# nnethercott/hannoy

Hardware: AMD Instinct MI355X
Metric: vectors indexed/sec (build) + recall@10, 1M x 768 Cosine M=16 efC=100 (higher is better)
Workload: dtype f32

## Files before the change

### hannoy_amd/csrc/hny_host.cpp

```cpp
#include "../../include/hannoy_amd.h"
#include "hny_internal.h"
#include "hny_rust_sort.h"

#include <malloc.h>
#include <algorithm>
#include <array>
#include <atomic>
#include <mutex>
#include <chrono>
#include <cmath>
#include <cstdarg>
#include <cstdio>
#include <cstdlib>
#include <cstring>
#include <functional>
#include <iterator>
#include <memory>
#include <numeric>
#include <string>
#include <thread>
#include <type_traits>
#include <utility>
#include <vector>

// ... 295 lines not shown
  bool gaps_done = false;
  bool from_update = false;
  uint64_t n_done0 = 0;
  uint32_t up_layers = 1;
  std::vector<uint32_t> entry_points;
  std::vector<uint64_t> rec_first;
  std::vector<uint32_t> rec_item_t;
  std::vector<uint8_t> rec_layer_t;
  std::vector<int32_t> upper_idx;
  uint32_t max_level = 0, n_upper = 0;
  LaunchShape shape{64, 1};
  double frac = 0.0;
  uint32_t bmax = 0;
  int device = 0;
  hipStream_t stream = nullptr;
  std::vector<hipEvent_t> sync_evs;
  size_t sync_used = 0;
  size_t pos = 0;
  uint64_t n_done = 0, n_batches = 0;
  hny_batch cur{};
  bool in_batch = false, finalized = false;
  GraphDev g{};
  DevBuf<unsigned char> d_rows, d_level;
  DevBuf<float> d_norms, d_l0_dist, d_up_dist;
  DevBuf<int> d_upper_idx;
  DevBuf<u32> d_l0_ids, d_l0_cnt, d_up_ids, d_up_cnt, d_order, d_eps, d_bits, d_vlog, d_cand_n,
      d_seg_start, d_nseg, d_deferred, d_deferred_b, d_fin_cnt0, d_fin_cntu, d_d0_ids, d_du_ids;
  DevBuf<unsigned char> d_has_vec, d_deleted;
  DevBuf<u64> d_old_recs, d_lkey_a, d_lkey_b, d_perm_a, d_perm_b;
  DevBuf<u32> d_gap_bitmap, d_gap_bm;
  DevBuf<u64> d_gap_keys, d_gap_sorted;
  int gap_grid = 0;
  DevBuf<u32> d_eps0;
  DevBuf<u32> d_pool_retry, d_pool_retry2, d_pool_ctr;
  DevBuf<u64> d_heap_c, d_heap_r;
  uint32_t heap_grid = 0, heap_c_cap = 0, heap_r_cap = 0, pool_ctr_used = 0;
  uint32_t heap_grid1 = 0, heap_c_cap1 = 0;
  u64 *heap_c_ptr = nullptr;
  struct ExportBufs : ExportSlots {
    std::thread th;
    void join() {
      if (th.joinable()) th.join();
    }
    void drop() {
      join();
      drop_all();
    }
    ~ExportBufs() { drop(); }
  } xbuf;
  bool will_export = true;
  std::vector<uint32_t> item_slot;
  uint64_t n_items = 0;
  std::unique_ptr<IngestPipe> qpipe;
  uint64_t nrec_bound = 0, nbr_bound = 0;
  bool locality = true;
  u32 *h_l0 = nullptr, *h_up = nullptr, *h_cnt0 = nullptr, *h_cntu = nullptr;
  DevBuf<u64> d_stats, d_stats_scratch, d_sel, d_cand, d_res_global;
  DevBuf<u64> d_ops;
  struct { u64 *p = nullptr; size_t n = 0; } d_keys_a, d_keys_b, d_vals_a, d_vals_b;
  DevBuf<unsigned char> d_sort_tmp;
  size_t sort_tmp_bytes = 0;
  uint32_t walk_slots = 0, bits_words = 0, log_cap = 0, rcap = 0, max_batch = 0;
  Knobs knobs{};
  uint32_t xcd_tile = 0, prune_xcd_tile = 0, walk_resident = 0;
  uint64_t top_layer_nodes = 0;
  StageRows stage{0, 0};
// ... 116 lines not shown
  for (uint32_t v : set)
    if (c <= v) {
      s.lpr = (int)l;
      s.nch = (int)v;
      return HNY_OK;
    }
  return fail(HNY_ERR_UNSUPPORTED, "dim %u needs more than 16 chunks per lane (max f32 dim 4096)", dim);
}

int mclass_of(int metric) {
  switch (metric) {
    case HNY_COSINE: return MC_DOT;
    case HNY_EUCLIDEAN: return MC_L2;
    case HNY_MANHATTAN: return MC_L1;
    default: return MC_BIN;
  }
}

uint32_t cap_of(const hny_builder *b, uint32_t layer_or_level) {
  return layer_or_level == 0 ? b->o.M0 : b->o.M;
}

int env_int(const char *name, int dflt) {
  const char *v = getenv(name);
  return v && *v ? atoi(v) : dflt;
}

Knobs knobs_from_env() {
  Knobs k{};
  k.no_fast = env_int("HNY_NO_FAST", 0) != 0;
  k.no_rb = env_int("HNY_NO_RB", 0) != 0;
  k.rb_one = env_int("HNY_RB_ONE", 1) != 0;
  k.prune_n8 = env_int("HNY_PRUNE_N8", 1) != 0;
  k.walk_slots = env_int("HNY_WALK_SLOTS", HNY_KNOB_UNSET);
  k.xcd_tile = env_int("HNY_XCD_TILE", HNY_KNOB_UNSET);
  k.prune_xcd_tile = env_int("HNY_PRUNE_XCD_TILE", HNY_KNOB_UNSET);
  k.walk_resident = env_int("HNY_WALK_RESIDENT", HNY_KNOB_UNSET);
  k.visited_log = env_int("HNY_VISITED_LOG", HNY_KNOB_UNSET);
  k.vis_slots = env_int("HNY_VIS_SLOTS", HNY_KNOB_UNSET);
  k.stage_bytes = env_int("HNY_STAGE_BYTES", HNY_KNOB_UNSET);
  k.no_locality = env_int("HNY_NO_LOCALITY", 0) != 0;
  k.heap_small_cap = env_int("HNY_HEAP_SMALL_CAP", HNY_KNOB_UNSET);
  k.vis_buckets = env_int("HNY_VIS_BUCKETS", HNY_KNOB_UNSET);
  return k;
}

int upload_rows(const void *vectors, size_t stride, size_t vbytes, uint64_t n, uint32_t row_stride,
                unsigned char *dst, hipStream_t st, const uint32_t *slots = nullptr, uint64_t n_slots = 0) {
  if (!slots) n_slots = n;
  if (!slots && stride == row_stride && vbytes == row_stride) {
    HIP_TRY(hipMemcpyAsync(dst, vectors, (size_t)n * row_stride, hipMemcpyHostToDevice, st));
    HIP_TRY(hipStreamSynchronize(st));
    return HNY_OK;
  }
  const size_t chunk_rows = std::max<size_t>(1, (64u << 20) / row_stride);
  std::vector<unsigned char> stage(chunk_rows * row_stride);
  uint64_t r = 0;
  for (uint64_t s0 = 0; s0 < n_slots; s0 += chunk_rows) {
    size_t cnt = (size_t)std::min<uint64_t>(chunk_rows, n_slots - s0);
    std::fill(stage.begin(), stage.begin() + cnt * row_stride, 0);
    for (; r < n && (slots ? slots[r] : r) < s0 + cnt; r++)
      memcpy(&stage[((slots ? slots[r] : r) - s0) * row_stride], (const unsigned char *)vectors + r * stride, vbytes);
    HIP_TRY(hipMemcpyAsync(dst + s0 * row_stride, stage.data(), cnt * row_stride,
                           hipMemcpyHostToDevice, st));
    HIP_TRY(hipStreamSynchronize(st));
  }
// ... 116 lines not shown
    if (j.out_codes)
      HIP_TRY(hipMemcpyAsync((unsigned char *)j.out_codes + r0 * vb, p.d_codes[k], (size_t)cnt * vb, hipMemcpyDeviceToHost, st));
    if (j.out_hdrs)
      HIP_TRY(hipMemcpyAsync((unsigned char *)j.out_hdrs + r0 * hb, p.d_hdrs[k], (size_t)cnt * hb, hipMemcpyDeviceToHost, st));
  }
  return HNY_OK;
}

int check_f32_rows(uint32_t dim, uint64_t n, const void *vectors, size_t stride) {
  if (dim == 0) return fail(HNY_ERR_INVALID_DIM, "dim must be > 0");
  if (n && !vectors) return fail(HNY_ERR_INVALID_ARG, "null f32 vectors");
  if (n && stride < (size_t)dim * 4)
    return fail(HNY_ERR_INVALID_DIM, "stride %zu < %zu bytes of f32 for dim %u", stride, (size_t)dim * 4, dim);
  if (n && stride % 4) return fail(HNY_ERR_INVALID_ARG, "f32 stride %zu is not a multiple of 4", stride);
  return HNY_OK;
}

int reset_graph(hny_builder *b) {
  hipStream_t st = b->stream;
  HIP_TRY(hnyk_fill_u32(b->d_l0_ids.p, HNY_SENT, b->d_l0_ids.n, st));
  HIP_TRY(hipMemsetAsync(b->d_l0_cnt.p, 0, b->d_l0_cnt.n * 4, st));
  HIP_TRY(hipMemsetAsync(b->d_l0_dist.p, 0, b->d_l0_dist.n * 4, st));
  if (b->d_up_ids.n) {
    HIP_TRY(hnyk_fill_u32(b->d_up_ids.p, HNY_SENT, b->d_up_ids.n, st));
    HIP_TRY(hipMemsetAsync(b->d_up_cnt.p, 0, b->d_up_cnt.n * 4, st));
    HIP_TRY(hipMemsetAsync(b->d_up_dist.p, 0, b->d_up_dist.n * 4, st));
  }
  HIP_TRY(hipMemsetAsync(b->d_stats.p, 0, ST_COUNT * 8, st));
  HIP_TRY(hipMemsetAsync(b->d_bits.p, 0, b->d_bits.n * 4, st));
  b->pos = 0;
  b->n_done = b->n_done0;
  b->n_batches = 0;
  b->in_batch = false;
  b->finalized = false;
  b->gaps_done = false;
  b->ev_used = 0;
  b->n_walk_dispatch = 0;
  b->sync_used = 0;
  b->t_build0 = now_s();
  return HNY_OK;
}

int use_device(int device) {
  int ndev = 0;
  if (hipGetDeviceCount(&ndev) != hipSuccess || ndev == 0)
    return fail(HNY_ERR_NO_DEVICE, "no HIP device (this library has no CPU path)");
  if (device >= 0) HIP_TRY(hipSetDevice(device));
  return HNY_OK;
}

size_t group_end(const hny_builder *b, size_t pos) {
  size_t e = pos;
  while (e < b->order.size() && b->order_level[e] == b->order_level[pos]) e++;
  return e;
}

inline uint32_t rec_mask_of(const hny_builder *b, uint32_t s) {
  if (b->deleted[s]) return 0u;
  uint32_t m = b->old_mask[s];
  if (b->ins_level[s] >= 0) m |= (2u << b->ins_level[s]) - 1u;
  return m;
}
template <class F>
inline void for_each_record(const hny_builder *b, uint32_t s, F &&fn) {
  for (uint32_t m = rec_mask_of(b, s), l = 0; m; m >>= 1, l++)
    if (m & 1) fn(l, l == 0 ? (size_t)s : (size_t)b->upper_idx[s] * b->up_layers + (l - 1));
// ... 618 lines not shown
}
static uint32_t walk_slots_default(const WalkForm &plain) { return 256u * 4u * (uint32_t)plain.waves_per_simd; }
static int plan_launch(hny_builder *b, const Knobs &knobs) {
  const hny_build_opts &o = b->o;
  const uint32_t n = b->n, n16 = b->g.n16;
  const Knobs &k = b->knobs = knobs;
  b->g.metric = o.metric;
  b->g.M = o.M;
  b->g.M0 = o.M0;
  b->g.incremental = b->incremental ? 1 : 0;
  b->g.x86_order = o.x86_order ? 1 : 0;
  b->rcap = res_capacity(o.ef_construction, (uint32_t)b->entry_points.size(), n, b->top_layer_nodes, HNY_RES_GLOBAL_MAX);
  b->rb_one = rb_one_of(o.ef_construction, b->entry_points.size(), b->top_layer_nodes, o.M);
  b->walk_slots = walk_slots_default(plain_walk_form(b, b->rcap, k.no_rb != 0));
  b->walk_slots = (uint32_t)std::min<int64_t>(std::max(1, knob_or(k.walk_slots, (int)b->walk_slots)), 65536);
  b->xcd_tile = (u32)std::max(0, knob_or(k.xcd_tile, n16 * 16u >= 1024u ? 512 : 0));
  b->prune_xcd_tile = (u32)std::max(0, knob_or(k.prune_xcd_tile, 512));
  const bool long_row_rb = n16 * 16u >= 1024u && plain_walk_form(b, b->rcap, false).rc != 0;
  const int resident = knob_or(k.walk_resident, long_row_rb ? 12 : 0);
  if (resident < 0 || resident > 256)
    return fail(HNY_ERR_INVALID_ARG, "HNY_WALK_RESIDENT=%d: 0 (= HNY_WALK_SLOTS) .. 256 waves per CU", resident);
  b->walk_resident = 256u * (u32)resident;
  b->bits_words = (n + 31) / 32 + 1;
  b->log_cap = (uint32_t)std::max(1024, knob_or(k.visited_log, 16384));
  b->locality = !k.no_locality;
  int rpg = 64 / b->shape.lpr;
  int sl = (int)((u32)std::max(0, knob_or(k.stage_bytes, 24576)) / (n16 * 16u));
  if (sl > HNY_MAX_CAP) sl = HNY_MAX_CAP;
  b->stage.wg = sl / rpg * rpg;
  b->stage.n8 = (int)std::min<uint32_t>(HNY_MAX_CAP, std::max<uint32_t>(1, 6144u / (n16 * 16u)));
  b->apply_form = hnyk_apply_form(b->g, b->shape, k);
  return HNY_OK;
}
static int plan_sizes(hny_builder *b, const CreatePlan &P) {
  const hny_build_opts &o = b->o;
  b->max_batch = 1;
  b->max_ops = 2;
  b->sel_words = 2;
  for (size_t pos = 0; pos < b->order.size();) {
    size_t e = group_end(b, pos);
    uint32_t L = b->order_level[pos];
    uint64_t bs = std::min<uint64_t>(b->bmax, e - pos);
    uint64_t cs = cap_of(b, L);
    b->max_batch = std::max<uint32_t>(b->max_batch, (uint32_t)bs);
    b->max_ops = std::max<size_t>(b->max_ops, (size_t)(bs * (L + 1) * cs * 2));
    b->sel_words = std::max<size_t>(b->sel_words, (size_t)(bs * (L + 1) * (cs + 1)));
    pos = e;
  }
  if (b->max_ops >= (1ull << HNY_SEQ_BITS))
    return fail(HNY_ERR_UNSUPPORTED,
                "batch_max %u too large for M0 %u: %zu link ops per batch >= 2^%d (pass batch_max <= %u; the schedule "
                "is part of the result, so it is never shrunk silently)",
                b->bmax, o.M0, b->max_ops, HNY_SEQ_BITS, (uint32_t)((1ull << (HNY_SEQ_BITS - 1)) / std::max(o.M0, 2 * o.M) / 2));
  if (int rc = plan_launch(b, knobs_from_env())) return rc;
  if (o.M0 > HNY_MAX_CAP && b->shape.nch > 8 && P.inc && !P.inc->load_only)
    return fail(HNY_ERR_UNSUPPORTED, "M0 %u > %d: an incremental build needs the workgroup kernels (rows <= 8 KB)",
                o.M0, HNY_MAX_CAP);
  return HNY_OK;
}

static int alloc_device(hny_builder *b, const CreatePlan &P) {
  const hny_build_opts &o = b->o;
  hipStream_t st = b->stream;
  const uint32_t n = b->n;
  const size_t nn = std::max<uint32_t>(n, 1);
  const size_t no = std::max<size_t>(b->order.size(), 1);
  const size_t nup = (size_t)b->n_upper * b->up_layers;
  const uint32_t row_stride = b->g.n16 * 16;
  HIP_TRY(b->d_rows.alloc(nn * row_stride));
  HIP_TRY(b->d_level.alloc(nn));
  HIP_TRY(b->d_upper_idx.alloc(nn));
  if (has_norms(o.metric)) HIP_TRY(b->d_norms.alloc(nn));
  HIP_TRY(b->d_l0_ids.alloc(nn * o.M0));
  HIP_TRY(b->d_l0_dist.alloc(nn * o.M0));
  HIP_TRY(b->d_l0_cnt.alloc(nn));
  HIP_TRY(b->d_up_ids.alloc(nup * o.M));
  HIP_TRY(b->d_up_dist.alloc(nup * o.M));
  HIP_TRY(b->d_up_cnt.alloc(nup));
  HIP_TRY(b->d_order.alloc(no));
  HIP_TRY(b->d_fin_cnt0.alloc(nn));
  HIP_TRY(b->d_fin_cntu.alloc(std::max<size_t>(nup, 1)));
  HIP_TRY(hipHostMalloc((void **)&b->h_l0, nn * o.M0 * 4));
  HIP_TRY(hipHostMalloc((void **)&b->h_cnt0, nn * 4));
  HIP_TRY(hipHostMalloc((void **)&b->h_up, std::max<size_t>(nup * o.M, 1) * 4));
  HIP_TRY(hipHostMalloc((void **)&b->h_cntu, std::max<size_t>(nup, 1) * 4));
  HIP_TRY(b->d_eps.alloc(std::max<size_t>(64, b->entry_points.size())));
  HIP_TRY(b->d_stats.alloc(ST_COUNT));
  const uint32_t slots = std::min<uint32_t>(b->walk_slots, std::max<uint32_t>(b->max_batch, 256));
  b->walk_slots = slots;
  HIP_TRY(b->d_bits.alloc((size_t)slots * b->bits_words));
  HIP_TRY(b->d_vlog.alloc((size_t)slots * b->log_cap));
  HIP_TRY(b->d_sel.alloc(b->sel_words));
  const size_t cand_rows = std::max<uint32_t>(b->max_batch, 256);
  if (b->rcap > HNY_RES_LDS_MAX) {
    if (b->apply_form.kind == APPLY_WAVE)
      return fail(HNY_ERR_UNSUPPORTED, "a result set of %u entries needs the workgroup prune kernels (no x86_order, rows <= 8 KB)", b->rcap);
    if ((cand_rows + slots) * (size_t)b->rcap * 8 > ((size_t)24 << 30))
      return fail(HNY_ERR_UNSUPPORTED, "result sets of %u entries for %zu batch members exceed the 24 GB set aside for them; "
                  "pass a smaller batch_max", b->rcap, cand_rows);
    HIP_TRY(b->d_res_global.alloc((size_t)slots * b->rcap));
  }
  HIP_TRY(b->d_cand.alloc(cand_rows * b->rcap));
  HIP_TRY(b->d_cand_n.alloc(cand_rows));
  HIP_TRY(b->d_ops.alloc(4 * b->max_ops));
  b->d_keys_a.p = b->d_ops.p;
  b->d_keys_b.p = b->d_ops.p + b->max_ops;
  b->d_vals_a.p = b->d_ops.p + 2 * b->max_ops;
  b->d_vals_b.p = b->d_ops.p + 3 * b->max_ops;
  b->d_keys_a.n = b->d_keys_b.n = b->d_vals_a.n = b->d_vals_b.n = b->max_ops;
  HIP_TRY(b->d_seg_start.alloc(b->max_ops));
  HIP_TRY(b->d_nseg.alloc(4 + 16 + 8 * 16));
  HIP_TRY(b->d_lkey_a.alloc(cand_rows));
  HIP_TRY(b->d_lkey_b.alloc(cand_rows));
  HIP_TRY(b->d_perm_a.alloc(cand_rows));
  HIP_TRY(b->d_perm_b.alloc(cand_rows));
  HIP_TRY(b->d_eps0.alloc(cand_rows));
  {
    const uint64_t c_full = (uint64_t)n + 1 + eps_cap_of(b);
    b->heap_r_cap = b->rcap + 1;
    if (b->d_ops.n >= c_full) {
      b->heap_c_cap = (uint32_t)std::min<uint64_t>(c_full, 0xFFFFFFFFull);
      b->heap_grid = (uint32_t)std::min<uint64_t>(std::min<uint64_t>(slots, 512), b->d_ops.n / c_full);
      b->heap_c_ptr = b->d_ops.p;
    } else {
      b->heap_c_cap = (uint32_t)std::min<uint64_t>(c_full, (uint64_t)1 << 25);
      b->heap_grid = (uint32_t)std::max<uint64_t>(1, std::min<uint64_t>(std::min<uint64_t>(slots, 512), ((uint64_t)1 << 25) / b->heap_c_cap));
      HIP_TRY(b->d_heap_c.alloc((size_t)b->heap_grid * b->heap_c_cap));
      b->heap_c_ptr = b->d_heap_c.p;
    }
    const uint64_t area = b->heap_c_ptr == b->d_ops.p ? b->d_ops.n : b->d_heap_c.n;
    const uint64_t small_cap = (uint64_t)std::max(16, knob_or(b->knobs.heap_small_cap, 1 << 18));
    if ((uint64_t)b->heap_c_cap > small_cap) {
      b->heap_c_cap1 = (uint32_t)small_cap;
      b->heap_grid1 = (uint32_t)std::max<uint64_t>(1, std::min<uint64_t>(std::min<uint64_t>(slots, 512), area / small_cap));
      HIP_TRY(b->d_pool_retry2.alloc(cand_rows));
    }
    HIP_TRY(b->d_heap_r.alloc((size_t)std::max(b->heap_grid, b->heap_grid1) * b->heap_r_cap));
    HIP_TRY(b->d_pool_retry.alloc(cand_rows));
    HIP_TRY(b->d_pool_ctr.alloc(4 * 64));
  }
  HIP_TRY(b->d_deferred.alloc(b->max_ops));
  HIP_TRY(b->d_deferred_b.alloc(b->max_ops));
  {
    u32 tbits = 1;
    while ((1ull << tbits) < (u64)b->n + 1ull) tbits++;
    const u32 ranges[3][2] = {{0, 64}, {HNY_SEQ_BITS, 64}, {HNY_SEQ_BITS, (u32)HNY_SEQ_BITS + tbits}};
    b->sort_tmp_bytes = 0;
    for (size_t sz = b->max_ops; sz >= 1; sz = sz > 1 ? sz / 2 : 0) {
      for (auto &r : ranges) {
        size_t need = 0;
        HIP_TRY(hnyk_sort_pairs(nullptr, need, b->d_keys_a.p, b->d_keys_b.p, b->d_vals_a.p, b->d_vals_b.p,
                                (u32)sz, r[0], r[1], st));
        b->sort_tmp_bytes = std::max(b->sort_tmp_bytes, need);
      }
      size_t need = 0;
      HIP_TRY(hnyk_sort_pairs48(nullptr, need, b->d_keys_a.p, b->d_keys_b.p, b->d_vals_a.p, b->d_vals_b.p,
                                (u32)sz, st));
      b->sort_tmp_bytes = std::max(b->sort_tmp_bytes, need);
      need = 0;
      HIP_TRY(hnyk_sort_u32(nullptr, need, b->d_deferred.p, b->d_deferred_b.p, (u32)sz, st));
      b->sort_tmp_bytes = std::max(b->sort_tmp_bytes, need);
      if (sz == 1) break;
    }
  }
  HIP_TRY(b->d_sort_tmp.alloc(b->sort_tmp_bytes + 16));
  if (b->incremental && n) {
    HIP_TRY(b->d_d0_ids.alloc((size_t)n * o.M0));
    HIP_TRY(b->d_du_ids.alloc(std::max<size_t>(nup * o.M, 1)));
    HIP_TRY(b->d_has_vec.alloc(n));
    HIP_TRY(b->d_deleted.alloc(n));
    HIP_TRY(b->d_old_recs.alloc(std::max<size_t>(b->old_recs.size(), 1)));
  }

  GraphDev &g = b->g;
  const size_t vb = vec_bytes(o.metric, o.dim);
  g.n = n;
  g.metric = o.metric;
  g.mclass = mclass_of(o.metric);
  g.row_stride = row_stride;
  g.bin_bits = (u32)(vb * 8);
  g.bin_inv = (g.bin_bits && (g.bin_bits & (g.bin_bits - 1)) == 0) ? 1.0f / (float)g.bin_bits : 0.0f;
  g.M = o.M;
  g.M0 = o.M0;
  g.max_level = b->max_level;
  g.up_layers = b->up_layers;
  g.n_upper = b->n_upper;
  g.alpha = o.alpha;
  g.incremental = b->incremental ? 1 : 0;
  g.dim = o.dim;
  g.x86_order = o.x86_order ? 1 : 0;
  g.rows = b->d_rows.p;
  g.norms = b->d_norms.p;
  g.level = b->d_level.p;
  g.upper_idx = b->d_upper_idx.p;
  g.l0_ids = b->d_l0_ids.p;
// ... 168 lines not shown
  for (uint32_t s0 = 0; s0 < b->n && i < b->n_items; s0 += (uint32_t)chunk) {
    const uint32_t cnt = (uint32_t)std::min<size_t>(chunk, b->n - s0);
    HIP_TRY(hipMemcpy(tmp.data(), b->d_rows.p + (size_t)s0 * rs, (size_t)cnt * rs, hipMemcpyDeviceToHost));
    for (; i < b->n_items && slot_of_item(i) < s0 + cnt; i++)
      memcpy((unsigned char *)out_codes + i * vb, &tmp[(size_t)(slot_of_item(i) - s0) * rs], vb);
  }
  if (b->n_items) memset(out_headers, 0, (size_t)b->n_items * hb);
  if (b->g.norms && b->n_items) {
    std::vector<float> norms(b->n);
    HIP_TRY(hipMemcpy(norms.data(), b->d_norms.p, (size_t)b->n * 4, hipMemcpyDeviceToHost));
    for (uint64_t k = 0; k < b->n_items; k++) memcpy((unsigned char *)out_headers + k * hb, &norms[slot_of_item(k)], 4);
  }
  return HNY_OK;
}

int hny_builder_reset(hny_builder *b) {
  if (!b) return fail(HNY_ERR_INVALID_ARG, "null builder");
  HIP_TRY(hipSetDevice(b->device));
  return reset_graph(b);
}

static void start_export_prefault(hny_builder *b);
int hny_builder_next_batch(hny_builder *b, hny_batch *out) {
  if (!b || !out) return fail(HNY_ERR_INVALID_ARG, "null argument");
  if (b->in_batch) return fail(HNY_ERR_INVALID_ARG, "previous batch not applied");
  if (b->finalized && b->pos < b->order.size()) return fail(HNY_ERR_INVALID_ARG, "graph already finalised");
  memset(out, 0, sizeof *out);
  if (b->pos >= b->order.size()) return HNY_OK;
  if (b->pos == 0) start_export_prefault(b);
  size_t gend = group_end(b, b->pos);
  uint32_t L = b->order_level[b->pos];
  uint64_t bs = hny_batch_size(b->frac, b->bmax, b->n_done);
  bs = std::min<uint64_t>(bs, gend - b->pos);
  out->first = b->pos;
  out->count = (uint32_t)bs;
  out->level = L;
  out->n_layers = L + 1;
  out->sel_stride_u64 = (L + 1) * (cap_of(b, L) + 1);
  b->cur = *out;
  b->in_batch = true;
  return HNY_OK;
}

static hipError_t next_sync_event(hny_builder *b, hipEvent_t *ev) {
  if (b->sync_used == b->sync_evs.size()) {
    hipEvent_t e;
    hipError_t rc = hipEventCreateWithFlags(&e, hipEventDisableTiming);
    if (rc != hipSuccess) return rc;
    b->sync_evs.push_back(e);
  }
  *ev = b->sync_evs[b->sync_used++];
  return hipSuccess;
}

static void walk_workspace(const hny_builder *b, WalkArgs &w, uint32_t rcap, u64 *res_global) {
  w.entry_points = b->d_eps.p;
  w.n_entry_points = (u32)b->entry_points.size();
  w.rcap = rcap;
  w.bits = b->d_bits.p;
  w.bits_words = b->bits_words;
  w.vlog = b->d_vlog.p;
  w.log_cap = b->log_cap;
  w.res_global = res_global;
  w.vis_slots = vis_slots_for(b, res_global ? 0u : rcap);
  w.eps_cap = eps_cap_of(b);
  vis_buckets_for(b, w);
}

static u32 xcd_tile_of(const hny_builder *b, uint32_t cnt) {
  return b->xcd_tile && cnt >= 16u * b->xcd_tile ? b->xcd_tile : 0u;
}

static int walk_resident_of(const hny_builder *b, uint32_t cnt) {
  const u32 slots = b->walk_resident ? std::min(b->walk_resident, b->walk_slots) : b->walk_slots;
  return (int)std::min<uint32_t>(cnt, slots);
}

static bool pool_retry_env(WalkArgs &w) {
  w.force_pool = (u32)std::max(0, env_int("HNY_POOL_FORCE_RETRY", 0));
  return env_int("HNY_NO_POOL_RETRY", 0) == 0;
}

static WalkArgs region_descent(const hny_builder *b, WalkArgs w) {
  w.descend_only = 1;
  w.eps_out = b->d_eps0.p;
  w.key_out = b->d_lkey_a.p;
  return w;
}
static int region_order(hny_builder *b, uint32_t lo, uint32_t cnt, WalkArgs &w) {
  HIP_TRY(hnyk_iota_u64(b->d_perm_a.p, lo, cnt, b->stream));
  size_t tmp = b->sort_tmp_bytes;
  HIP_TRY(hnyk_sort_pairs48(b->d_sort_tmp.p, tmp, b->d_lkey_a.p, b->d_lkey_b.p, b->d_perm_a.p, b->d_perm_b.p, cnt,
                            b->stream));
  w.first = 0;
  w.eps_in = b->d_eps0.p;
  w.perm = b->d_perm_b.p;
  return HNY_OK;
}

int hny_builder_search(hny_builder *b, uint32_t lo, uint32_t hi, void *sel_dev) {
  if (!b || !b->in_batch) return fail(HNY_ERR_INVALID_ARG, "no current batch");
  if (lo > hi || hi > b->cur.count) return fail(HNY_ERR_INVALID_ARG, "bad member range");
  if (lo == hi) return HNY_OK;
  HIP_TRY(hipSetDevice(b->device));
  const uint32_t L = b->cur.level, cs = cap_of(b, L);
  u64 *sel = sel_dev ? (u64 *)sel_dev : b->d_sel.p;
  auto walk_args = [&](int32_t l, uint32_t clo, uint32_t chi, u32 *queue) {
    WalkArgs w{};
    w.q_slots = b->d_order.p + b->cur.first;
    w.lo = clo;
    w.hi = chi;
    w.layer = (u32)l;
    w.ef = b->o.ef_construction;
    w.first = (l == (int32_t)L);
    w.reader_mode = 0;
    w.sel = sel;
    w.sel_stride = b->cur.sel_stride_u64;
    w.cap_sel = cs;
    w.batch_level = L;
    w.cand = b->d_cand.p;
    w.cand_n = b->d_cand_n.p;
    w.queue = queue;
    walk_workspace(b, w, b->rcap, b->d_res_global.p);
    w.rb_one = b->rb_one;
    return w;
  };
  auto prune_args = [&](int32_t l, uint32_t clo, uint32_t chi) {
    PruneArgs p{};
    p.q_slots = b->d_order.p + b->cur.first;
    p.lo = clo;
    p.hi = chi;
    p.layer = (u32)l;
    p.cap = cs;
    p.cand = b->d_cand.p;
    p.cand_n = b->d_cand_n.p;
    p.rcap = b->rcap;
// ... 20 lines not shown
      if (e != hipSuccess) return e;
      b->pool_ctr_used = 0;
    }
    u32 *pc = b->d_pool_ctr.p + b->pool_ctr_used;
    b->pool_ctr_used += 4;
    const bool no_retry = !pool_retry_env(w);
    w.pool_retry = no_retry ? nullptr : b->d_pool_retry.p;
    w.n_pool_retry = pc;
    const int grid = w.xcd_tile && w.layer == 0u ? walk_resident_of(b, w.hi - w.lo)
                                                 : (int)std::min<uint32_t>(w.hi - w.lo, b->walk_slots);
    hipError_t e = hnyk_walk(b->g, w, b->shape, hnyk_walk_form(b->g, w, b->shape, b->knobs), grid, st);
    if (e != hipSuccess || no_retry) return e;
    WalkArgs h = w;
    h.queue = pc + 1;
    h.xcd_tile = 0;
    h.heap_c = b->heap_c_ptr;
    h.heap_r = b->d_heap_r.p;
    h.heap_c_cap = b->heap_c_cap;
    h.heap_r_cap = b->heap_r_cap;
    if (b->heap_grid1) {
      WalkArgs h1 = h;
      h1.heap_c_cap = b->heap_c_cap1;
      h1.pool_retry2 = b->d_pool_retry2.p;
      h1.n_pool_retry2 = pc + 2;
      e = hnyk_walk_heap(b->g, h1, b->shape, (int)std::min<uint32_t>(w.hi - w.lo, b->heap_grid1), st);
      if (e != hipSuccess) return e;
      h.pool_retry = b->d_pool_retry2.p;
      h.n_pool_retry = pc + 2;
      h.queue = pc + 3;
    }
    return hnyk_walk_heap(b->g, h, b->shape, (int)std::min<uint32_t>(w.hi - w.lo, b->heap_grid), st);
  };

  const uint32_t cnt = hi - lo;
  if (b->locality && b->max_level > L && cnt >= 2048) {
    WalkArgs top = walk_args(L, lo, hi, queues + (L + 1));
    prof_begin(b, EV_WALK);
    b->n_walk_dispatch++;
    HIP_TRY(launch_walk(region_descent(b, walk_args(L, lo, hi, queues + 0)), b->stream));
    if (int rc = region_order(b, lo, cnt, top)) return rc;
    const u32 xcd_tile = xcd_tile_of(b, cnt);
    for (int32_t l = (int32_t)L; l >= 0; l--) {
      WalkArgs w = l == (int32_t)L ? top : walk_args(l, lo, hi, queues + (l + 1));
      w.perm = top.perm;
      if (l != (int32_t)L) prof_begin(b, EV_WALK);
      if (xcd_tile) {
        w.xcd_tile = xcd_tile;
        w.queue = xqueues + 8 * (l + 1);
      }
      b->n_walk_dispatch++;
      HIP_TRY(launch_walk(w, b->stream));
      prof_end(b);
      PruneArgs p = prune_args(l, lo, hi);
      p.perm = b->d_perm_b.p;
      prof_begin(b, EV_PRUNE);
      HIP_TRY(launch_prune(p, b->stream));
      prof_end(b);
    }
    return HNY_OK;
  }
  for (int32_t l = (int32_t)L; l >= 0; l--) {
    WalkArgs w = walk_args(l, lo, hi, queues + l);
    prof_begin(b, EV_WALK);
    b->n_walk_dispatch++;
    HIP_TRY(launch_walk(w, b->stream));
    prof_end(b);
    prof_begin(b, EV_PRUNE);
    HIP_TRY(launch_prune(prune_args(l, lo, hi), b->stream));
    prof_end(b);
  }
  return HNY_OK;
}

static int apply_front(hny_builder *b, const void *sel_dev, ApplyArgs &a) {
  const uint32_t L = b->cur.level, cs = cap_of(b, L);
  const u64 *sel = sel_dev ? (const u64 *)sel_dev : b->d_sel.p;
  const u32 n_ops = b->cur.count * (L + 1) * cs * 2;
  EmitArgs e{};
  e.q_slots = b->d_order.p + b->cur.first;
  e.count = b->cur.count;
  e.sel = sel;
  e.sel_stride = b->cur.sel_stride_u64;
  e.cap_sel = cs;
  e.batch_level = L;
  e.keys = b->d_keys_a.p;
  e.vals = b->d_vals_a.p;
  prof_begin(b, EV_SORT);
// ... 2631 lines not shown
```

### hannoy_amd/csrc/hny_internal.h

```cpp
#pragma once
#include <hip/hip_runtime.h>
#include <stddef.h>
#include <stdint.h>

typedef unsigned long long u64;
typedef unsigned int u32;

#define HNY_SENT 0xFFFFFFFFu
#define HNY_MAX_CAP 64
#define HNY_BIG_CAP 1024
#define HNY_MAX_EPS 8192
#define HNY_POOL_CAP 128
#define HNY_MAX_EF 65535
#define HNY_OP_INVALID 0xFFFFFFFFFFFFFFFFull
#define HNY_SEQ_BITS 29
#define HNY_MAX_LEVEL 14

enum { MC_DOT = 0, MC_L2 = 1, MC_L1 = 2, MC_BIN = 3 };

enum {
  ST_EVALS_WALK = 0,
  ST_EVALS_PRUNE = 1,
  ST_EVALS_APPLY = 2,
  ST_LINKS = 3,
// ... 142 lines not shown
struct EmitArgs {
  const u32 *q_slots;
  u32 count;
  const u64 *sel;
  u32 sel_stride, cap_sel, batch_level;
  u64 *keys;
  u64 *vals;
};

struct ApplyArgs {
  const u64 *keys;
  const u64 *vals;
  u32 n_ops;
  const u32 *seg_start;
  const u32 *n_seg;
  u32 *deferred;
  u32 *n_deferred;
  u32 shard_rank, shard_world;
  u64 *exch;
  u32 exch_stride;
};

struct LaunchShape {
  int lpr;
  int nch;
};

#define HNY_KNOB_UNSET (-2147483647 - 1)
struct Knobs {
  int no_fast;
  int no_rb;
  int rb_one;
  int prune_n8;
  int walk_slots, xcd_tile, prune_xcd_tile, walk_resident, visited_log, vis_slots, stage_bytes, no_locality,
      heap_small_cap, vis_buckets;
};
static inline int knob_or(int v, int dflt) { return v == HNY_KNOB_UNSET ? dflt : v; }

#ifndef HNY_RB_MAX_NCH
#define HNY_RB_MAX_NCH 3
#endif
#ifndef HNY_WALK_WPE
#define HNY_WALK_WPE 4
#endif
#ifndef HNY_WALK_WPE_SMALL
#define HNY_WALK_WPE_SMALL 6
#endif
constexpr int hnyk_walk_waves_per_simd(int lpr, int nch, int sp, bool rm, int rc) {
  return nch == 1 && sp >= 4 && !rm && (rc == 1 || rc == 2) && lpr <= 32 ? HNY_WALK_WPE_SMALL : HNY_WALK_WPE;
}

static inline bool hnyk_fast_path(const GraphDev &g, const Knobs &k) {
  return !k.no_fast && !g.x86_order && !g.incremental && g.metric >= 0 && g.metric < 7 && g.M0 <= 64u;
}
struct WalkForm {
  int sp;
  bool big_eps;
  bool reader;
  int rc;
  int waves_per_simd;
};
static inline WalkForm hnyk_walk_form(const GraphDev &g, const WalkArgs &a, LaunchShape s, const Knobs &k) {
  WalkForm f{0, a.eps_cap > 64, false, 0, 0};
  if (hnyk_fast_path(g, k) && a.eps_cap <= 64 && !a.res_global) {
    f.sp = g.metric + 1;
    f.reader = a.reader_mode != 0;
// ... 95 lines not shown
hipError_t hnyk_exact_topk(const GraphDev &g, const ExactArgs &a, hipStream_t st);
hipError_t hnyk_exact_tile_masks(const ExactArgs &a, hipStream_t st);
struct RangeArgs {
  const float *scores;
  u32 score_stride;
  u32 nq;
  u32 slab_base, slab_n;
  const u32 *mask;
  const float *radius;
  u64 *count;
  u64 *keys;
  const u32 *seg;
  u32 *cursor;
};
hipError_t hnyk_range_count(const RangeArgs &a, hipStream_t st);
hipError_t hnyk_range_emit(const RangeArgs &a, hipStream_t st);
hipError_t hnyk_range_sort(void *temp, size_t &temp_bytes, u64 *keys, u64 *other, u32 n, u32 n_seg, const u32 *seg,
                           u64 **sorted, hipStream_t st);
hipError_t hnyk_range_finish(const u64 *keys, u32 n, const u32 *item_ids, u32 *ids, u32 *dist_bits, hipStream_t st);
hipError_t hnyk_emit(const GraphDev &g, const EmitArgs &a, hipStream_t st);
hipError_t hnyk_segments(const u64 *keys, u32 n_ops, u32 *seg_start, u32 *n_seg, hipStream_t st);
hipError_t hnyk_apply(const GraphDev &g, const ApplyArgs &a, LaunchShape s, const ApplyForm &f, int grid, hipStream_t st);
hipError_t hnyk_apply_append(const GraphDev &g, const ApplyArgs &a, hipStream_t st);
hipError_t hnyk_apply_deferred(const GraphDev &g, const ApplyArgs &a, LaunchShape s, const ApplyForm &f, StageRows sl,
                               u32 work, hipStream_t st);
hipError_t hnyk_apply_merge(const GraphDev &g, const u64 *exch, u32 n_def, u32 world, u32 rank, u32 per,
                            u32 stride, hipStream_t st);
hipError_t hnyk_sort_u32(void *temp, size_t &temp_bytes, u32 *in, u32 *out, u32 n, hipStream_t st);
hipError_t hnyk_sort_pairs(void *temp, size_t &temp_bytes, u64 *keys_in, u64 *keys_out, u64 *vals_in,
                           u64 *vals_out, u32 n, u32 begin_bit, u32 end_bit, hipStream_t st);
hipError_t hnyk_sort_pairs48(void *temp, size_t &temp_bytes, u64 *keys_in, u64 *keys_out, u64 *vals_in,
                             u64 *vals_out, u32 n, hipStream_t st);
hipError_t hnyk_iota_u64(u64 *p, u32 base, u32 n, hipStream_t st);
hipError_t hnyk_take_topk(const u64 *cand, const u32 *cand_n, u32 rcap, u32 k, u32 n, u64 *out,
                          hipStream_t st);
hipError_t hnyk_lane_selftest(u32 *out64, hipStream_t st);
hipError_t hnyk_pair_distances(const GraphDev &g, const u32 *a, const u32 *b, u32 n, float *out,
                               LaunchShape s, hipStream_t st);
hipError_t hnyk_fill_u32(u32 *p, u32 v, size_t n, hipStream_t st);
hipError_t hnyk_fill_gaps_wg(const GraphDev &g, const u64 *recs, u32 n_recs, const unsigned char *deleted,
                             u32 *bitmaps, u32 words, u32 *bm, u32 maxb, u64 *keys, u64 *sorted, int SL, int grid,
                             LaunchShape s, hipStream_t st);
hipError_t hnyk_fill_gaps(const GraphDev &g, const u64 *recs, u32 n_recs, const unsigned char *deleted,
                          LaunchShape s, hipStream_t st);
hipError_t hnyk_finalize_lists(u32 *ids, u32 *cnt_out, u32 n_lists, u32 cap, hipStream_t st);
size_t hnyk_walk_lds_bytes(u32 rcap, u32 eps_cap);
#define HNY_DECL_SP(N)                                                                                         \
  hipError_t hnyk_walk_sp##N(const GraphDev &g, const WalkArgs &a, LaunchShape s, const WalkForm &f, int grid, \
                             hipStream_t st);                                                                  \
  hipError_t hnyk_prune_sp##N(const GraphDev &g, const PruneArgs &a, LaunchShape s, const PruneForm &f, int SL, \
                              int grid, hipStream_t st);                                                       \
  hipError_t hnyk_apply_sp##N(const GraphDev &g, const ApplyArgs &a, LaunchShape s, const ApplyForm &f, int SL, \
                              int grid, hipStream_t st);
HNY_DECL_SP(1) HNY_DECL_SP(2) HNY_DECL_SP(3) HNY_DECL_SP(4) HNY_DECL_SP(5) HNY_DECL_SP(6) HNY_DECL_SP(7)
#undef HNY_DECL_SP

enum { ING_F32 = 0, ING_F32_NORM = 1, ING_BINARY = 2, ING_BQ = 3 };
struct IngestArgs {
  const float *src;
  u32 src_stride, dim, cnt;
  const u32 *src_of;
  int codec;
  float hdr_const;
  const u32 *slots;
  u32 slot_base;
  unsigned char *rows;
// ... 47 lines not shown
```

### hannoy_amd/csrc/hny_kernels.hip

```cpp
#include "hny_internal.h"

#include <algorithm>
#include <cstdlib>
#include <cstring>
#ifndef HNY_PART
#define HNY_PART 0
#endif
#if HNY_PART == 0
#include <rocprim/device/device_radix_sort.hpp>
#endif

#ifdef HNY_WSYNC_BARRIER
#define WSYNC() __syncthreads()
#else
#define WSYNC()                                               \
  do {                                                        \
    __builtin_amdgcn_fence(__ATOMIC_RELEASE, "workgroup");    \
    __builtin_amdgcn_wave_barrier();                          \
    __builtin_amdgcn_fence(__ATOMIC_ACQUIRE, "workgroup");    \
  } while (0)
#endif

#ifndef HNY_RB_MERGE
#define HNY_RB_MERGE 1
// ... 4270 lines not shown
  if (!n_def || world < 2) return hipSuccess;
  hipLaunchKernelGGL(k_apply_merge, dim3(std::min<u32>(n_def, 8192u)), dim3(64), 0, st, g, exch, n_def, world,
                     rank, per, stride);
  return hipGetLastError();
}
hipError_t hnyk_sort_pairs48(void *temp, size_t &temp_bytes, u64 *keys_in, u64 *keys_out, u64 *vals_in,
                             u64 *vals_out, u32 n, hipStream_t st) {
  return rocprim::radix_sort_pairs(temp, temp_bytes, keys_in, keys_out, vals_in, vals_out, (size_t)n,
                                   0, 48, st);
}
__global__ void k_take_topk(const u64 *cand, const u32 *cand_n, u32 rcap, u32 k, u32 n, u64 *out) {
  u64 i = (u64)blockIdx.x * blockDim.x + threadIdx.x;
  if (i >= (u64)n * k) return;
  u32 q = (u32)(i / k), j = (u32)(i % k);
  out[i] = j < cand_n[q] ? cand[(size_t)q * rcap + j] : HNY_OP_INVALID;
}
hipError_t hnyk_take_topk(const u64 *cand, const u32 *cand_n, u32 rcap, u32 k, u32 n, u64 *out,
                          hipStream_t st) {
  u64 total = (u64)n * k;
  if (!total) return hipSuccess;
  hipLaunchKernelGGL(k_take_topk, dim3((unsigned)((total + 255) / 256)), dim3(256), 0, st, cand, cand_n,
                     rcap, k, n, out);
  return hipGetLastError();
}
__global__ void k_iota_u64(u64 *p, u32 base, u32 n) {
  u32 i = blockIdx.x * blockDim.x + threadIdx.x;
  if (i < n) p[i] = (u64)(base + i);
}
hipError_t hnyk_iota_u64(u64 *p, u32 base, u32 n, hipStream_t st) {
  if (!n) return hipSuccess;
  hipLaunchKernelGGL(k_iota_u64, dim3((n + 255) / 256), dim3(256), 0, st, p, base, n);
  return hipGetLastError();
}

template <int OFF>
__device__ __forceinline__ u32 lane_selftest_one(u32 v, u32 w) {
  u32 bad = 0;
  if (xshfl_u32<OFF>(v) != (u32)__shfl_xor((int)v, OFF, 64)) bad |= 1u;
  const bool hi = (threadIdx.x & OFF) != 0;
  {
    const u32 keep = hi ? w : v, send = hi ? v : w;
    if (fold_step<OFF, u32>(v, w) != keep + (u32)__shfl_xor((int)send, OFF, 64)) bad |= 2u;
  }
  {
    const float a = __uint_as_float(0x3F800000u | (v & 0x7FFFFFu)), b = __uint_as_float(0x40000000u | (w & 0x7FFFFFu));
    const float keep = hi ? b : a, send = hi ? a : b;
    const float ref = keep + __shfl_xor(send, OFF, 64);
    if (__float_as_uint(fold_step<OFF, float>(a, b)) != __float_as_uint(ref)) bad |= 4u;
    if (__float_as_uint(xshfl<OFF>(a)) != __float_as_uint(__shfl_xor(a, OFF, 64))) bad |= 8u;
  }
  const u64 q = ((u64)v << 32) | w;
  if (xshfl<OFF>(q) != (u64)__shfl_xor((long long)q, OFF, 64)) bad |= 16u;
  return bad;
}
__global__ __launch_bounds__(64) void k_lane_selftest(u32 *out) {
  const u32 v = (threadIdx.x + 1u) * 2654435761u, w = (threadIdx.x + 77u) * 40503u + 0x9E3779B9u;
  u32 bad = 0;
  bad |= lane_selftest_one<1>(v, w) << 0;
  bad |= lane_selftest_one<2>(v, w) << 5;
  bad |= lane_selftest_one<4>(v, w) << 10;
  bad |= lane_selftest_one<8>(v, w) << 15;
  bad |= lane_selftest_one<16>(v, w) << 20;
  bad |= lane_selftest_one<32>(v, w) << 25;
  out[threadIdx.x] = bad;
}
hipError_t hnyk_lane_selftest(u32 *out64, hipStream_t st) {
// ... 5 lines not shown
```

Measured before the change: 2.575 million.

## Run upper-layer descent once per level group and sort keys per batch

When a level group spans several batches, the build now runs the descend-only walk for every member of the group in a single launch. It then tags each member's locality key with its batch index and does one radix sort that gives per-batch permutations. Later batches in the group reuse the stored entry points and permutations instead of running their own descent and region ordering. This cuts the number of kernel launches and sorts. The cost is larger key and permutation buffers sized to the biggest group, a host-to-device copy of the batch starts, and extra bookkeeping that is reset whenever a partial or mismatched batch shows up.

```diff
diff --git a/hannoy_amd/csrc/hny_host.cpp b/hannoy_amd/csrc/hny_host.cpp
--- a/hannoy_amd/csrc/hny_host.cpp
+++ b/hannoy_amd/csrc/hny_host.cpp
@@ -351,6 +351,14 @@
   DevBuf<u64> d_gap_keys, d_gap_sorted;
   int gap_grid = 0;
   DevBuf<u32> d_eps0;
+  struct GroupDescent {
+    bool planned = false, done = false;
+    size_t first = 0;
+    std::vector<u32> starts;
+  } grp;
+  size_t group_cap = 0;
+  DevBuf<u32> d_geps, d_gstart;
+  DevBuf<u64> d_gperm;
   DevBuf<u32> d_pool_retry, d_pool_retry2, d_pool_ctr;
   DevBuf<u64> d_heap_c, d_heap_r;
   uint32_t heap_grid = 0, heap_c_cap = 0, heap_r_cap = 0, pool_ctr_used = 0;
@@ -533,6 +541,7 @@
   k.no_rb = env_int("HNY_NO_RB", 0) != 0;
   k.rb_one = env_int("HNY_RB_ONE", 1) != 0;
   k.prune_n8 = env_int("HNY_PRUNE_N8", 1) != 0;
+  k.group_descent = env_int("HNY_GROUP_DESCENT", 1) != 0;
   k.walk_slots = env_int("HNY_WALK_SLOTS", HNY_KNOB_UNSET);
   k.xcd_tile = env_int("HNY_XCD_TILE", HNY_KNOB_UNSET);
   k.prune_xcd_tile = env_int("HNY_PRUNE_XCD_TILE", HNY_KNOB_UNSET);
@@ -715,6 +724,7 @@
   b->n_done = b->n_done0;
   b->n_batches = 0;
   b->in_batch = false;
+  b->grp = {};
   b->finalized = false;
   b->gaps_done = false;
   b->ev_used = 0;
@@ -1399,6 +1409,10 @@
   b->apply_form = hnyk_apply_form(b->g, b->shape, k);
   return HNY_OK;
 }
+static bool group_descent_allowed(const hny_builder *b, uint32_t L, size_t members, uint64_t most_per_batch) {
+  return b->knobs.group_descent && b->locality && !b->incremental && !b->o.x86_order && b->max_level > L &&
+         b->bmax != 1 && members >= 2048 && members > most_per_batch && members < (1ull << 31);
+}
 static int plan_sizes(hny_builder *b, const CreatePlan &P) {
   const hny_build_opts &o = b->o;
   b->max_batch = 1;
@@ -1420,6 +1434,13 @@
                 "is part of the result, so it is never shrunk silently)",
                 b->bmax, o.M0, b->max_ops, HNY_SEQ_BITS, (uint32_t)((1ull << (HNY_SEQ_BITS - 1)) / std::max(o.M0, 2 * o.M) / 2));
   if (int rc = plan_launch(b, knobs_from_env())) return rc;
+  b->group_cap = 0;
+  for (size_t pos = 0; pos < b->order.size();) {
+    size_t e = group_end(b, pos);
+    if (group_descent_allowed(b, b->order_level[pos], e - pos, hny_batch_size(b->frac, b->bmax, pos)))
+      b->group_cap = std::max(b->group_cap, e - pos);
+    pos = e;
+  }
   if (o.M0 > HNY_MAX_CAP && b->shape.nch > 8 && P.inc && !P.inc->load_only)
     return fail(HNY_ERR_UNSUPPORTED, "M0 %u > %d: an incremental build needs the workgroup kernels (rows <= 8 KB)",
                 o.M0, HNY_MAX_CAP);
@@ -1477,11 +1498,17 @@
   b->d_keys_a.n = b->d_keys_b.n = b->d_vals_a.n = b->d_vals_b.n = b->max_ops;
   HIP_TRY(b->d_seg_start.alloc(b->max_ops));
   HIP_TRY(b->d_nseg.alloc(4 + 16 + 8 * 16));
-  HIP_TRY(b->d_lkey_a.alloc(cand_rows));
-  HIP_TRY(b->d_lkey_b.alloc(cand_rows));
-  HIP_TRY(b->d_perm_a.alloc(cand_rows));
+  const size_t key_rows = std::max(cand_rows, b->group_cap);
+  HIP_TRY(b->d_lkey_a.alloc(key_rows));
+  HIP_TRY(b->d_lkey_b.alloc(key_rows));
+  HIP_TRY(b->d_perm_a.alloc(key_rows));
   HIP_TRY(b->d_perm_b.alloc(cand_rows));
   HIP_TRY(b->d_eps0.alloc(cand_rows));
+  if (b->group_cap) {
+    HIP_TRY(b->d_geps.alloc(b->group_cap));
+    HIP_TRY(b->d_gperm.alloc(b->group_cap));
+    HIP_TRY(b->d_gstart.alloc(65536 + 1));
+  }
   {
     const uint64_t c_full = (uint64_t)n + 1 + eps_cap_of(b);
     b->heap_r_cap = b->rcap + 1;
@@ -1500,10 +1527,10 @@
     if ((uint64_t)b->heap_c_cap > small_cap) {
       b->heap_c_cap1 = (uint32_t)small_cap;
       b->heap_grid1 = (uint32_t)std::max<uint64_t>(1, std::min<uint64_t>(std::min<uint64_t>(slots, 512), area / small_cap));
-      HIP_TRY(b->d_pool_retry2.alloc(cand_rows));
+      HIP_TRY(b->d_pool_retry2.alloc(key_rows));
     }
     HIP_TRY(b->d_heap_r.alloc((size_t)std::max(b->heap_grid, b->heap_grid1) * b->heap_r_cap));
-    HIP_TRY(b->d_pool_retry.alloc(cand_rows));
+    HIP_TRY(b->d_pool_retry.alloc(key_rows));
     HIP_TRY(b->d_pool_ctr.alloc(4 * 64));
   }
   HIP_TRY(b->d_deferred.alloc(b->max_ops));
@@ -1513,7 +1540,7 @@
     while ((1ull << tbits) < (u64)b->n + 1ull) tbits++;
     const u32 ranges[3][2] = {{0, 64}, {HNY_SEQ_BITS, 64}, {HNY_SEQ_BITS, (u32)HNY_SEQ_BITS + tbits}};
     b->sort_tmp_bytes = 0;
-    for (size_t sz = b->max_ops; sz >= 1; sz = sz > 1 ? sz / 2 : 0) {
+    for (size_t sz = std::max(b->max_ops, b->group_cap); sz >= 1; sz = sz > 1 ? sz / 2 : 0) {
       for (auto &r : ranges) {
         size_t need = 0;
         HIP_TRY(hnyk_sort_pairs(nullptr, need, b->d_keys_a.p, b->d_keys_b.p, b->d_vals_a.p, b->d_vals_b.p,
@@ -1528,6 +1555,11 @@
       HIP_TRY(hnyk_sort_u32(nullptr, need, b->d_deferred.p, b->d_deferred_b.p, (u32)sz, st));
       b->sort_tmp_bytes = std::max(b->sort_tmp_bytes, need);
       if (sz == 1) break;
+    }
+    if (b->group_cap) {
+      size_t need = 0;
+      HIP_TRY(hnyk_sort_pairs(nullptr, need, b->d_lkey_a.p, b->d_lkey_b.p, b->d_perm_a.p, b->d_gperm.p, (u32)b->group_cap, 0, 64, st));
+      b->sort_tmp_bytes = std::max(b->sort_tmp_bytes, need);
     }
   }
   HIP_TRY(b->d_sort_tmp.alloc(b->sort_tmp_bytes + 16));
@@ -1762,6 +1794,22 @@
   uint32_t L = b->order_level[b->pos];
   uint64_t bs = hny_batch_size(b->frac, b->bmax, b->n_done);
   bs = std::min<uint64_t>(bs, gend - b->pos);
+  if (b->pos == 0 || b->order_level[b->pos - 1] != L) {
+    b->grp = {};
+    const size_t members = gend - b->pos;
+    if (members <= b->group_cap && group_descent_allowed(b, L, members, bs)) {
+      uint64_t done = b->n_done;
+      for (size_t p = b->pos; p < gend;) {
+        b->grp.starts.push_back((u32)(p - b->pos));
+        const uint64_t c = std::min<uint64_t>(hny_batch_size(b->frac, b->bmax, done), gend - p);
+        p += c;
+        done += c;
+      }
+      b->grp.starts.push_back((u32)members);
+      b->grp.first = b->pos;
+      b->grp.planned = b->grp.starts.size() - 1 <= 65536;
+    }
+  }
   out->first = b->pos;
   out->count = (uint32_t)bs;
   out->level = L;
@@ -1828,10 +1876,18 @@
   return HNY_OK;
 }
 
+static int search_batch(hny_builder *b, uint32_t lo, uint32_t hi, void *sel_dev);
 int hny_builder_search(hny_builder *b, uint32_t lo, uint32_t hi, void *sel_dev) {
   if (!b || !b->in_batch) return fail(HNY_ERR_INVALID_ARG, "no current batch");
   if (lo > hi || hi > b->cur.count) return fail(HNY_ERR_INVALID_ARG, "bad member range");
   if (lo == hi) return HNY_OK;
+  if ((lo != 0 || hi != b->cur.count) && !b->grp.done) b->grp = {};
+  const int rc = search_batch(b, lo, hi, sel_dev);
+  if (rc != HNY_OK) b->grp = {};
+  return rc;
+}
+
+static int search_batch(hny_builder *b, uint32_t lo, uint32_t hi, void *sel_dev) {
   HIP_TRY(hipSetDevice(b->device));
   const uint32_t L = b->cur.level, cs = cap_of(b, L);
   u64 *sel = sel_dev ? (u64 *)sel_dev : b->d_sel.p;
@@ -1918,13 +1974,55 @@
     return hnyk_walk_heap(b->g, h, b->shape, (int)std::min<uint32_t>(w.hi - w.lo, b->heap_grid), st);
   };
 
+  auto group_descent = [&](WalkArgs w) -> int {
+    const u32 members = b->grp.starts.back(), n_batches = (u32)b->grp.starts.size() - 1;
+    w.lo = 0;
+    w.hi = members;
+    w.descend_only = 1;
+    w.eps_out = b->d_geps.p;
+    w.key_out = b->d_lkey_a.p;
+    HIP_TRY(launch_walk(w, b->stream));
+    HIP_TRY(hipMemcpyAsync(b->d_gstart.p, b->grp.starts.data(), b->grp.starts.size() * 4, hipMemcpyHostToDevice, b->stream));
+    HIP_TRY(hnyk_group_keys(b->d_lkey_a.p, b->d_perm_a.p, b->d_gstart.p, n_batches, members, b->stream));
+    size_t tmp = b->sort_tmp_bytes;
+    HIP_TRY(hnyk_sort_pairs(b->d_sort_tmp.p, tmp, b->d_lkey_a.p, b->d_lkey_b.p, b->d_perm_a.p, b->d_gperm.p, members, 0, 64,
+                            b->stream));
+    b->grp.done = true;
+    return HNY_OK;
+  };
+
   const uint32_t cnt = hi - lo;
-  if (b->locality && b->max_level > L && cnt >= 2048) {
+  int64_t gbatch = -1;
+  if (b->grp.planned && b->cur.first >= b->grp.first) {
+    const u32 off = (u32)(b->cur.first - b->grp.first);
+    auto it = std::lower_bound(b->grp.starts.begin(), b->grp.starts.end() - 1, off);
+    if (it != b->grp.starts.end() - 1 && *it == off && it[1] - off == b->cur.count && (b->grp.done || off == 0))
+      gbatch = it - b->grp.starts.begin();
+  }
+  if (b->grp.planned && gbatch < 0) b->grp = {};
+  if (gbatch >= 0 || (b->locality && b->max_level > L && cnt >= 2048)) {
     WalkArgs top = walk_args(L, lo, hi, queues + (L + 1));
     prof_begin(b, EV_WALK);
-    b->n_walk_dispatch++;
-    HIP_TRY(launch_walk(region_descent(b, walk_args(L, lo, hi, queues + 0)), b->stream));
-    if (int rc = region_order(b, lo, cnt, top)) return rc;
+    if (gbatch >= 0) {
+      if (!b->grp.done) {
+        b->n_walk_dispatch++;
+        if (int rc = group_descent(walk_args(L, lo, hi, queues + 0))) return rc;
+      }
+      top.first = 0;
+      top.eps_in = b->d_geps.p + b->grp.starts[gbatch];
+      top.perm = b->d_gperm.p + b->grp.starts[gbatch];
+      if (cnt != b->cur.count) {
+        HIP_TRY(hnyk_iota_u64(b->d_perm_a.p, lo, cnt, b->stream));
+        size_t tmp = b->sort_tmp_bytes;
+        HIP_TRY(hnyk_sort_pairs48(b->d_sort_tmp.p, tmp, b->d_lkey_a.p + b->grp.starts[gbatch] + lo, b->d_lkey_b.p,
+                                  b->d_perm_a.p, b->d_perm_b.p, cnt, b->stream));
+        top.perm = b->d_perm_b.p;
+      }
+    } else {
+      b->n_walk_dispatch++;
+      HIP_TRY(launch_walk(region_descent(b, walk_args(L, lo, hi, queues + 0)), b->stream));
+      if (int rc = region_order(b, lo, cnt, top)) return rc;
+    }
     const u32 xcd_tile = xcd_tile_of(b, cnt);
     for (int32_t l = (int32_t)L; l >= 0; l--) {
       WalkArgs w = l == (int32_t)L ? top : walk_args(l, lo, hi, queues + (l + 1));
@@ -1938,7 +2036,7 @@
       HIP_TRY(launch_walk(w, b->stream));
       prof_end(b);
       PruneArgs p = prune_args(l, lo, hi);
-      p.perm = b->d_perm_b.p;
+      p.perm = top.perm;
       prof_begin(b, EV_PRUNE);
       HIP_TRY(launch_prune(p, b->stream));
       prof_end(b);
diff --git a/hannoy_amd/csrc/hny_internal.h b/hannoy_amd/csrc/hny_internal.h
--- a/hannoy_amd/csrc/hny_internal.h
+++ b/hannoy_amd/csrc/hny_internal.h
@@ -198,6 +198,7 @@
   int no_rb;
   int rb_one;
   int prune_n8;
+  int group_descent;
   int walk_slots, xcd_tile, prune_xcd_tile, walk_resident, visited_log, vis_slots, stage_bytes, no_locality,
       heap_small_cap, vis_buckets;
 };
@@ -359,6 +360,7 @@
 hipError_t hnyk_sort_pairs48(void *temp, size_t &temp_bytes, u64 *keys_in, u64 *keys_out, u64 *vals_in,
                              u64 *vals_out, u32 n, hipStream_t st);
 hipError_t hnyk_iota_u64(u64 *p, u32 base, u32 n, hipStream_t st);
+hipError_t hnyk_group_keys(u64 *keys, u64 *vals, const u32 *starts, u32 n_batches, u32 n, hipStream_t st);
 hipError_t hnyk_take_topk(const u64 *cand, const u32 *cand_n, u32 rcap, u32 k, u32 n, u64 *out,
                           hipStream_t st);
 hipError_t hnyk_lane_selftest(u32 *out64, hipStream_t st);
diff --git a/hannoy_amd/csrc/hny_kernels.hip b/hannoy_amd/csrc/hny_kernels.hip
--- a/hannoy_amd/csrc/hny_kernels.hip
+++ b/hannoy_amd/csrc/hny_kernels.hip
@@ -4326,6 +4326,23 @@
   hipLaunchKernelGGL(k_iota_u64, dim3((n + 255) / 256), dim3(256), 0, st, p, base, n);
   return hipGetLastError();
 }
+__global__ void k_group_keys(u64 *keys, u64 *vals, const u32 *starts, u32 n_batches, u32 n) {
+  u32 i = blockIdx.x * blockDim.x + threadIdx.x;
+  if (i >= n) return;
+  u32 lo = 0, hi = n_batches;
+  while (hi - lo > 1u) {
+    const u32 mid = (lo + hi) / 2u;
+    if (starts[mid] <= i) lo = mid;
+    else hi = mid;
+  }
+  keys[i] = ((u64)lo << 48) | (keys[i] & 0xFFFFFFFFFFFFull);
+  vals[i] = (u64)(i - starts[lo]);
+}
+hipError_t hnyk_group_keys(u64 *keys, u64 *vals, const u32 *starts, u32 n_batches, u32 n, hipStream_t st) {
+  if (!n) return hipSuccess;
+  hipLaunchKernelGGL(k_group_keys, dim3((n + 255) / 256), dim3(256), 0, st, keys, vals, starts, n_batches, n);
+  return hipGetLastError();
+}
 
 template <int OFF>
 __device__ __forceinline__ u32 lane_selftest_one(u32 v, u32 w) {
```

Result: no change. 2.594 million, median of 6 (+0.7%).
